# Pitt-JonesLab/slam_decomposition

Hardware: AMD Instinct MI355X
Metric: Haar 2-qubit decompositions/sec (span<=3, loss<1e-8) (higher is better)
Workload: dtype f64

## Files before the change

slam_decomposition_amd/csrc/slam_device.hpp:

```cpp
#pragma once
#include <hip/hip_runtime.h>
#include <stdint.h>

#include "slam_sincos.hpp"
#include "slam_types.hpp"

namespace slamdev {

constexpr int kQuadsPerWave = 16;
constexpr int kWave = 64;
constexpr int kRow = kWave + 1;

typedef float f32x2 __attribute__((ext_vector_type(2)));
typedef float f32x4 __attribute__((ext_vector_type(4)));

template <int K, bool PSQ = false>
struct Cfg {
    static constexpr int L = K + 1;
    static constexpr int N = 6 * L;
    static constexpr int NA = (N + 3) / 4;
    static constexpr int NP = NA * 4;
    static constexpr int NBLK = NA * (NA + 1) / 2;
    static constexpr int FNEED = 20 * NA - 16;
    static constexpr int FSTRIDE = (FNEED - 4 + 31) / 32 * 32 + 4;
    static constexpr int PSP = (N + 3) / 4 * 4 + 1;
    static constexpr int TOFF = PSQ ? 6 : 0;
    static constexpr int PS0 = 12 * K + TOFF;
    static constexpr int XNEED_D = PSQ ? PS0 + 3 * PSP + N : 2 * N;
    static constexpr int XNEED_F = (kQuadsPerWave * FSTRIDE + 2 * kQuadsPerWave - 1) / (2 * kQuadsPerWave);
    static constexpr int XNEED = XNEED_D > XNEED_F ? XNEED_D : XNEED_F;
    static constexpr int XSTRIDE = PSQ ? (XNEED - 4 + 15) / 16 * 16 + 4 : (XNEED - 4 + 7) / 8 * 8 + 4;
    static constexpr int LDS_XCHG = kQuadsPerWave * XSTRIDE;
    static_assert(kQuadsPerWave * FSTRIDE * 4 <= LDS_XCHG * 8, "float overlay must fit the exchange area");
    static constexpr int LDS_FH = 2 * K * 4 * kRow * 2;
    static constexpr int LDS_DOUBLES = LDS_XCHG + LDS_FH;
    static constexpr int LDS_FH_LEAN = (K - 1) * 4 * kRow * 2;
    static constexpr int LDS_DOUBLES_LEAN = LDS_XCHG + LDS_FH_LEAN;
};

template <int K, int GC>
__host__ __device__ constexpr bool lean_layout() { return GC != 0; }
template <int K, int GC>
__host__ __device__ constexpr bool psq_layout() { return lean_layout<K, GC>() && K <= 3; }
template <int K, int GC>
__host__ __device__ constexpr int lds_work_doubles() {
    return lean_layout<K, GC>() ? Cfg<K, psq_layout<K, GC>()>::LDS_DOUBLES_LEAN : Cfg<K, false>::LDS_DOUBLES;
}
constexpr int kColdDoubles = 4;
constexpr int kSincosLdsDoubles = 2 * kSincosTableDoubles;
constexpr int kSeedRing = 8;
constexpr int kSeedRingOff = 70;
template <int K, int GC>
__host__ __device__ constexpr bool seed_ring() { return K == 1 && psq_layout<K, GC>(); }
template <int K, int GC>
__host__ __device__ constexpr int lds_doubles() { return lds_work_doubles<K, GC>() + kSincosLdsDoubles + kColdDoubles; }

__device__ const double kSinCosTable[kSincosTableDoubles] = SLAM_SINCOS_TABLE;

__device__ __forceinline__ void load_sincos_table(double2* tbl, int lane) {
    const double2 t = reinterpret_cast<const double2*>(kSinCosTable)[lane & 31];
    tbl[lane] = (lane & 32) ? make_double2(-t.x, -t.y) : t;
}

typedef const __attribute__((address_space(4))) double* gate_ptr;

__device__ __forceinline__ gate_ptr gate_matrix(const double* gates, int j) {
    unsigned long long a = (unsigned long long)(gates + 32 * j);
    asm volatile("" : "+s"(a));
    return (gate_ptr)a;
}

template <int CTRL>
__device__ __forceinline__ double dpp_f64(double v) {
    int lo = __double2loint(v), hi = __double2hiint(v);
    lo = __builtin_amdgcn_update_dpp(0, lo, CTRL, 0xF, 0xF, true);
    hi = __builtin_amdgcn_update_dpp(0, hi, CTRL, 0xF, 0xF, true);
    return __hiloint2double(hi, lo);
}
template <int CTRL>
__device__ __forceinline__ int dpp_i32(int v) {
    return __builtin_amdgcn_update_dpp(0, v, CTRL, 0xF, 0xF, true);
}
template <int CTRL>
__device__ __forceinline__ double quad_shuffle(double v) { return dpp_f64<CTRL>(v); }
__device__ __forceinline__ double quad_sum(double v) {
    v += quad_shuffle<0xB1>(v);
    v += quad_shuffle<0x4E>(v);
    return v;
}
__device__ __forceinline__ void quad_sum2(double& a, double& b) {
    const double a1 = quad_shuffle<0xB1>(a), b1 = quad_shuffle<0xB1>(b);
    a += a1; b += b1;
    const double a2 = quad_shuffle<0x4E>(a), b2 = quad_shuffle<0x4E>(b);
    a += a2; b += b2;
}
__device__ __forceinline__ double max_abs(double a, double b) {
    double m;
    asm("v_max_f64 %0, |%1|, |%2|" : "=v"(m) : "v"(a), "v"(b));
    return m;
}
__device__ __forceinline__ double quad_max(double v) {
    v = max_abs(v, quad_shuffle<0xB1>(v));
    v = max_abs(v, quad_shuffle<0x4E>(v));
    return v;
}

__device__ __forceinline__ void lds_fence() {
    __builtin_amdgcn_fence(__ATOMIC_RELEASE, "wavefront");
    __builtin_amdgcn_wave_barrier();
    __builtin_amdgcn_fence(__ATOMIC_ACQUIRE, "wavefront");
}

__device__ __forceinline__ void philox4x32_10(uint32_t c0, uint32_t c1, uint32_t c2, uint32_t c3,
                                              uint32_t k0, uint32_t k1, uint32_t (&out)[4]) {
#pragma unroll
    for (int r = 0; r < 10; ++r) {
        const uint64_t p0 = (uint64_t)0xD2511F53u * c0;
        const uint64_t p1 = (uint64_t)0xCD9E8D57u * c2;
        const uint32_t n0 = (uint32_t)(p1 >> 32) ^ c1 ^ k0;
        const uint32_t n1 = (uint32_t)p1;
        const uint32_t n2 = (uint32_t)(p0 >> 32) ^ c3 ^ k1;
        const uint32_t n3 = (uint32_t)p0;
        c0 = n0; c1 = n1; c2 = n2; c3 = n3;
        k0 += 0x9E3779B9u;
        k1 += 0xBB67AE85u;
    }
    out[0] = c0; out[1] = c1; out[2] = c2; out[3] = c3;
}

__device__ __forceinline__ double x0_from_words(uint32_t a, uint32_t b) {
    const uint64_t m = ((uint64_t)(a >> 5) << 26) + (uint64_t)(b >> 6);
    return (double)m * (1.0 / 9007199254740992.0) * 6.283185307179586476925286766559;
}
__device__ __forceinline__ double x0_philox(uint64_t seed, uint32_t target, uint32_t restart, uint32_t k,
                                            uint32_t i) {
    uint32_t w[4];
    philox4x32_10(i >> 1, restart, target, k, (uint32_t)seed, (uint32_t)(seed >> 32), w);
    return (i & 1) ? x0_from_words(w[2], w[3]) : x0_from_words(w[0], w[1]);
}

struct U3t {
    double c, s;
    double cp, sp;
    double cl, sl;
};

__device__ __forceinline__ U3t load_u3(const double* xq, int base_param) {
    const double2* t = reinterpret_cast<const double2*>(xq) + base_param;
    const double2 a = t[0], b = t[1], c = t[2];
    U3t u;
    u.c = a.x; u.s = a.y; u.cp = b.x; u.sp = b.y; u.cl = c.x; u.sl = c.y;
    return u;
}

__device__ __forceinline__ void u3_col(const U3t& t, double& f0r, double& f0i, double& f1r, double& f1i) {
    const double g1r = t.cl * f1r - t.sl * f1i;
    const double g1i = t.cl * f1i + t.sl * f1r;
    const double y0r = t.c * f0r - t.s * g1r;
    const double y0i = t.c * f0i - t.s * g1i;
    const double tr = t.s * f0r + t.c * g1r;
    const double ti = t.s * f0i + t.c * g1i;
    f0r = y0r; f0i = y0i;
    f1r = t.cp * tr - t.sp * ti;
    f1i = t.cp * ti + t.sp * tr;
}

__device__ __forceinline__ void u3_unit(const U3t& t, double f0, double f1, double& y0r, double& y0i, double& y1r, double& y1i) {
    const double g1r = t.cl * f1, g1i = t.sl * f1;
    y0r = t.c * f0 - t.s * g1r;
    y0i = -(t.s * g1i);
    const double tr = t.s * f0 + t.c * g1r;
    const double ti = t.c * g1i;
    y1r = t.cp * tr - t.sp * ti;
    y1i = t.cp * ti + t.sp * tr;
}

__device__ __forceinline__ void u3_unit_t(const U3t& t, double f0, double f1, double& y0r, double& y0i, double& y1r, double& y1i,
                                          double& tr, double& ti) {
// ... 408 lines not shown
        mr[p] = (xr[a] * zr[b] - xi[a] * zi[b]) - (xr[b] * zr[a] - xi[b] * zi[a]);
        mi[p] = (xr[a] * zi[b] + xi[a] * zr[b]) - (xr[b] * zi[a] + xi[b] * zr[a]);
    }
#pragma unroll
    for (int p = 0; p < 6; ++p) { orr[p] = dpp_f64<0x4E>(mr[p]); oi[p] = dpp_f64<0x4E>(mi[p]); }
    const bool hi = q & 2;
    double dr = 0.0, di = 0.0;
#pragma unroll
    for (int p = 0; p < 6; ++p) {
        const double Pr = hi ? orr[p] : mr[p], Pi = hi ? oi[p] : mi[p];
        const double Qr = hi ? mr[5 - p] : orr[5 - p], Qi = hi ? mi[5 - p] : oi[5 - p];
        const double s = (p == 1 || p == 4) ? -1.0 : 1.0;
        dr = fma(s, Pr * Qr - Pi * Qi, dr);
        di = fma(s, Pr * Qi + Pi * Qr, di);
    }
    v.dr = dr; v.di = di;
}

__device__ __forceinline__ void mk_g(const MkInv& v, double (&g)[3], double& idr, double& idi, double& G1r, double& G1i, double& G2r,
                                     double& G2i) {
    const double rd = fast_rcp(v.dr * v.dr + v.di * v.di);
    idr = v.dr * rd; idi = -v.di * rd;
    const double sr = v.tr * v.tr - v.ti * v.ti, si = 2.0 * v.tr * v.ti;
    G1r = 0.0625 * (sr * idr - si * idi); G1i = 0.0625 * (sr * idi + si * idr);
    const double er = sr - v.t2r, ei = si - v.t2i;
    G2r = 0.25 * (er * idr - ei * idi); G2i = 0.25 * (er * idi + ei * idr);
    g[0] = G1r; g[1] = G1i; g[2] = G2r;
}

__device__ __forceinline__ void mk_target_g(const double* tcol, int q, double (&g)[3]) {
    double tr[4], ti[4];
#pragma unroll
    for (int r = 0; r < 4; ++r) {
        const double2 t = *reinterpret_cast<const double2*>(tcol + 8 * r);
        tr[r] = t.x; ti[r] = t.y;
    }
    MkInv v;
    mk_invariants(tr, ti, q, v);
    double a, b, c, d, e, f;
    mk_g(v, g, a, b, c, d, e, f);
}

__device__ __forceinline__ void mk_loss_seed(const double (&wr)[4], const double (&wi)[4], int q, const double (&gT)[3], double& fout,
                                             double (&Ur)[4], double (&Ui)[4]) {
    MkInv v;
    mk_invariants(wr, wi, q, v);
    double g[3], idr, idi, G1r, G1i, G2r, G2i;
    mk_g(v, g, idr, idi, G1r, G1i, G2r, G2i);
    const double D1 = g[0] - gT[0], D2 = g[1] - gT[1], D3 = g[2] - gT[2];
    fout = fma(D1, D1, fma(D2, D2, D3 * D3));
    const double a1r = 2.0 * D1, a1i = -2.0 * D2, a3 = 2.0 * D3;
    const double tdr = v.tr * idr - v.ti * idi, tdi = v.tr * idi + v.ti * idr;
    const double cr = fma(0.125, a1r, 0.5 * a3), ci = 0.125 * a1i;
    const double alr = tdr * cr - tdi * ci, ali = tdr * ci + tdi * cr;
    const double ber = -0.25 * a3 * idr, bei = -0.25 * a3 * idi;
    const double gar = -((a1r * G1r - a1i * G1i) + a3 * G2r), gai = -((a1r * G1i + a1i * G1r) + a3 * G2i);
    double accr[4] = {0.0, 0.0, 0.0, 0.0}, acci[4] = {0.0, 0.0, 0.0, 0.0};
    auto accum = [&](int m, const double (&cr_)[4], const double (&ci_)[4]) {
        const double kr = mk_y(m) * v.br[3 - m], ki = mk_y(m) * v.bi[3 - m];
#pragma unroll
        for (int r = 0; r < 4; ++r) {
            accr[r] = fma(kr, cr_[r], fma(-ki, ci_[r], accr[r]));
            acci[r] = fma(kr, ci_[r], fma(ki, cr_[r], acci[r]));
        }
    };
    { double c0r[4], c0i[4]; mk_bcast_col<0>(wr, wi, c0r, c0i); accum(0, c0r, c0i); }
    { double c1r[4], c1i[4]; mk_bcast_col<1>(wr, wi, c1r, c1i); accum(1, c1r, c1i); }
    { double c2r[4], c2i[4]; mk_bcast_col<2>(wr, wi, c2r, c2i); accum(2, c2r, c2i); }
    { double c3r[4], c3i[4]; mk_bcast_col<3>(wr, wi, c3r, c3i); accum(3, c3r, c3i); }
    double wbr[4], wbi[4];
#pragma unroll
    for (int r = 0; r < 4; ++r) { wbr[r] = dpp_f64<0x1B>(wr[r]); wbi[r] = dpp_f64<0x1B>(wi[r]); }
    const double yq = ((q + 1) & 2) ? 1.0 : -1.0;
#pragma unroll
    for (int c = 0; c < 4; ++c) {
        const double s = yq * mk_y(c);
        const double xr = 2.0 * (alr * wbr[3 - c] - ali * wbi[3 - c]) + 4.0 * (ber * accr[3 - c] - bei * acci[3 - c]);
        const double xi = 2.0 * (alr * wbi[3 - c] + ali * wbr[3 - c]) + 4.0 * (ber * acci[3 - c] + bei * accr[3 - c]);
        Ur[c] = fma(s, xr, gar * wr[c] + gai * wi[c]);
        Ui[c] = fma(s, xi, gai * wr[c] - gar * wi[c]);
    }
}

template <int K, bool HUGE_ARGS, int GC, bool MK = false, bool ROOMY = false>
__device__ __forceinline__ void eval_quad(const double (&xd)[Cfg<K>::NA], const double* tcol,
                                          const double* gates, double* xq, double2* fh, const double2* tbl,
                                          int q, int theta_bits, int cost_kind, double& fout, double (&gd)[Cfg<K>::NA],
                                          double (&Wr)[4], double (&Wi)[4], const double* mkt = nullptr,
                                          const EvalLaneConsts<Cfg<K>::NA>* lc = nullptr) {
    constexpr bool LEAN = lean_layout<K, GC>();
    constexpr bool PSQ = psq_layout<K, GC>();
    using C = Cfg<K, PSQ>;
    static_assert(!ROOMY || (!HUGE_ARGS && !MK), "the hoisted lane constants: the optimizer's BasicCost / SquareCost evaluation only");
    if constexpr (!ROOMY) asm volatile("" : "+v"(theta_bits));
    double* const xt = xq + (PSQ ? (int)((threadIdx.x & 4) + ((threadIdx.x >> 2) & 2)) : 0);
    auto HS = [](int j) constexpr { return LEAN ? j : 2 * j + 1; };
    double tre[4], tim[4];
    if constexpr (!MK) {
#pragma unroll
        for (int r = 0; r < 4; ++r) {
            const double2 t = *reinterpret_cast<const double2*>(tcol + 8 * r);
            tre[r] = t.x;
            tim[r] = t.y;
        }
    }
    {
        double2* t2 = reinterpret_cast<double2*>(xt);
        if constexpr (HUGE_ARGS) {
#pragma unroll
            for (int a = 0; a < C::NA; ++a) {
                const int i = 4 * a + q;
                const int i3 = i - 3 * ((i * 43) >> 7);
                const double arg = (i3 == 0) ? 0.5 * xd[a] : xd[a];
                double s, c;
                sincos_any(arg, tbl, s, c);
                t2[i] = make_double2(c, s);
            }
        } else {
            double rr[C::NA];
            int kk[C::NA];
            double2 tt[C::NA];
            SincosLits L = sincos_lits_device();
            if constexpr (ROOMY) { L.s1 = lc->s1; L.c1 = lc->c1; }
#pragma unroll
            for (int a = 0; a < C::NA; ++a) {
                int hexp;
                if constexpr (ROOMY) hexp = lc->hexp[a];
                else hexp = __builtin_amdgcn_sbfe(theta_bits, a, 1);
                const double arg = __builtin_amdgcn_ldexp(xd[a], hexp);
                sincos_tbl_lookup<true>(arg, tbl, L, rr[a], kk[a], tt[a]);
            }
            __builtin_amdgcn_sched_barrier(0);
#pragma unroll
            for (int a = 0; a < C::NA; ++a) {
                double s, c;
                sincos_tbl_finish<true>(rr[a], kk[a], tt[a], L, s, c);
                t2[4 * a + q] = make_double2(c, s);
            }
        }
    }
    lds_fence();

    double Pr[4], Pi[4];
    double e0[2], e1[2];
    if constexpr (ROOMY) {
        e0[0] = lc->e0[0]; e0[1] = lc->e0[1];
        e1[0] = lc->e1[0]; e1[1] = lc->e1[1];
    } else {
        int qo = q;
        asm volatile("" : "+v"(qo));
        e0[0] = (qo & 1) ? 0.0 : 1.0; e0[1] = (qo & 1) ? 1.0 : 0.0;
        e1[0] = (qo & 2) ? 0.0 : 1.0; e1[1] = (qo & 2) ? 1.0 : 0.0;
    }
    double Fr[4], Fi[4];
#pragma unroll
    for (int r = 0; r < 4; ++r) {
        Fr[r] = (r == q) ? 1.0 : 0.0;
        Fi[r] = 0.0;
    }
    U3t Bn = load_u3(xt, 0), An = load_u3(xt, 3);
#pragma unroll
    for (int j = 0; j <= K; ++j) {
        if (j > 0 && !LEAN) {
#pragma unroll
            for (int r = 0; r < 4; ++r) fh[((2 * (j - 1)) * 4 + r) * kRow] = make_double2(Fr[r], Fi[r]);
        }
        const U3t B = Bn;
        const U3t A = An;
        GateRegs<GC> Gf;
        if (j < K) {
            if constexpr (GC == GC_XRI || GC == GC_XRI1) u3_arrived(B, A);
            Gf = load_gate<GC>(gates, j);
            if constexpr (GC == GC_XRI || GC == GC_XRI1) __builtin_amdgcn_sched_barrier(0);
        }
        double b0r, b0i, b1r, b1i;
        if (j == 0) {
            u3_unit(B, e0[0], e0[1], b0r, b0i, b1r, b1i);
        } else {
            u3_col(B, Fr[0], Fi[0], Fr[1], Fi[1]);
            u3_col(B, Fr[2], Fi[2], Fr[3], Fi[3]);
        }
        if (j < K) {
            Bn = load_u3(xt, 6 * (j + 1));
            An = load_u3(xt, 6 * (j + 1) + 3);
            __builtin_amdgcn_sched_barrier(0);
        }
        if (j == 0) {
            double a0r, a0i, a1r, a1i;
            u3_unit(A, e1[0], e1[1], a0r, a0i, a1r, a1i);
            Fr[0] = a0r * b0r - a0i * b0i; Fi[0] = a0r * b0i + a0i * b0r;
            Fr[1] = a0r * b1r - a0i * b1i; Fi[1] = a0r * b1i + a0i * b1r;
            Fr[2] = a1r * b0r - a1i * b0i; Fi[2] = a1r * b0i + a1i * b0r;
            Fr[3] = a1r * b1r - a1i * b1i; Fi[3] = a1r * b1i + a1i * b1r;
        } else {
            u3_col(A, Fr[0], Fi[0], Fr[2], Fi[2]);
            u3_col(A, Fr[1], Fi[1], Fr[3], Fi[3]);
        }
        if (j < K) {
            if (LEAN && j == K - 1) {
#pragma unroll
                for (int r = 0; r < 4; ++r) { Pr[r] = Fr[r]; Pi[r] = Fi[r]; }
            } else {
#pragma unroll
                for (int r = 0; r < 4; ++r) fh[(HS(j) * 4 + r) * kRow] = make_double2(Fr[r], Fi[r]);
            }
            gate_col<GC>(Gf, Fr, Fi);
        }
    }
#pragma unroll
    for (int r = 0; r < 4; ++r) { Wr[r] = Fr[r]; Wi[r] = Fi[r]; }

    double Ur[4], Ui[4];
    if constexpr (MK) {
        const double gT[3] = {mkt[0], mkt[1], mkt[2]};
        mk_loss_seed(Fr, Fi, q, gT, fout, Ur, Ui);
    } else {
        double pr = 0.0, pi = 0.0;
#pragma unroll
        for (int r = 0; r < 4; ++r) {
            pr = fma(tre[r], Fr[r], fma(tim[r], Fi[r], pr));
            pi = fma(tre[r], Fi[r], fma(-tim[r], Fr[r], pi));
        }
        quad_sum2(pr, pi);
        const double at2 = pr * pr + pi * pi;
        const double rat = (at2 > 1e-300) ? fast_rsqrt(at2) : 0.0;
        const double at = at2 * rat;
        const double basic = 1.0 - 0.25 * at;
        asm volatile("" : "+s"(cost_kind));
        const bool sq = (cost_kind == 1);
        double c0;
        if constexpr (ROOMY) c0 = lc->c0;
        else c0 = sq ? 1.6 : 1.0;
        const double c1 = sq ? -0.8 : 0.0, d1 = sq ? -1.6 : 0.0;
        fout = basic * fma(c1, basic, c0);
        const double inv = (0.25 * rat) * fma(d1, basic, c0);
        const double zr = -pr * inv, zi = pi * inv;
#pragma unroll
        for (int r = 0; r < 4; ++r) {
            Ur[r] = zr * tre[r] + zi * tim[r];
            Ui[r] = zi * tre[r] - zr * tim[r];
        }
    }

// ... 86 lines not shown
            dtheta_dlam_last_real(B, Ur[0], Ui[0], tB01r, tB01i, fr[0], fr[1], th01, la01);
            dtheta_dlam_last_real(B, Ur[2], Ui[2], tB23r, tB23i, fr[2], fr[3], th23, la23);
        }
        part[0] = th01 + th23;
        part[2] = la01 + la23;
        if (j > 0) {
            const double l2 = im_mul(Ur[2], Ui[2], fr[2], fi[2]);
            const double l3 = im_mul(Ur[3], Ui[3], fr[3], fi[3]);
            part[5] = -(l2 + l3);
        } else {
            part[5] = -(Ui[2] * fr[2] + Ui[3] * fr[3]);
        }
        if constexpr (kThetaOut)
            part[3] = 0.5 * thA2;
        else
            part[3] = dtheta_pair(A, Ur[0], Ui[0], Ur[2], Ui[2], fr[0], fi[0], fr[2], fi[2]) +
                      dtheta_pair(A, Ur[1], Ui[1], Ur[3], Ui[3], fr[1], fi[1], fr[3], fi[3]);
        if (kBwdTrigAhead && j > 0) {
            Bn = load_u3(xt, 6 * (j - 1));
            An = load_u3(xt, 6 * (j - 1) + 3);
            __builtin_amdgcn_sched_barrier(0);
        }
        if constexpr (PSQ) {
#pragma unroll
            for (int m = 0; m < 6; ++m) xq[C::PS0 + q * C::PSP + 6 * j + m] = part[m];
        } else {
#pragma unroll
            for (int m = 0; m < 6; ++m) {
                const double ps = part[m] + dpp_f64<0xB1>(part[m]);
                if ((q & 1) == 0) xq[12 * j + 2 * m + (q >> 1)] = ps;
            }
        }
        if (!kBwdTrigAhead && j > 0) {
            An = load_u3(xt, 6 * (j - 1) + 3);
            Bn = load_u3(xt, 6 * (j - 1));
            __builtin_amdgcn_sched_barrier(0);
        }
        if (j > 0) {
            gate_row<GC>(Gb, Ur, Ui);
            if (LEAN) {
#pragma unroll
                for (int r = 0; r < 4; ++r) { Hr[r] = Pr[r]; Hi[r] = Pi[r]; }
            }
        }
    }

    if constexpr (kL0Out) {
        const U3t B = Bn;
        const U3t A = An;
        double b0r, b0i, b1r, b1i, tbr, tbi, a0r, a0i, a1r, a1i, tar, tai;
        u3_unit_t(B, e0[0], e0[1], b0r, b0i, b1r, b1i, tbr, tbi);
        u3_unit_t(A, e1[0], e1[1], a0r, a0i, a1r, a1i, tar, tai);
        const double wB0r = (Ur[0] * a0r - Ui[0] * a0i) + (Ur[2] * a1r - Ui[2] * a1i), wB0i = (Ur[0] * a0i + Ui[0] * a0r) + (Ur[2] * a1i + Ui[2] * a1r);
        const double wB1r = (Ur[1] * a0r - Ui[1] * a0i) + (Ur[3] * a1r - Ui[3] * a1i), wB1i = (Ur[1] * a0i + Ui[1] * a0r) + (Ur[3] * a1i + Ui[3] * a1r);
        const double wA0r = (Ur[0] * b0r - Ui[0] * b0i) + (Ur[1] * b1r - Ui[1] * b1i), wA0i = (Ur[0] * b0i + Ui[0] * b0r) + (Ur[1] * b1i + Ui[1] * b1r);
        const double wA1r = (Ur[2] * b0r - Ui[2] * b0i) + (Ur[3] * b1r - Ui[3] * b1i), wA1i = (Ur[2] * b0i + Ui[2] * b0r) + (Ur[3] * b1i + Ui[3] * b1r);
        double part[6];
        l0_gate_partials(B, e0[0], e0[1], wB0r, wB0i, wB1r, wB1i, b0r, b0i, b1r, b1i, tbr, tbi, part[0], part[1], part[2]);
        l0_gate_partials(A, e1[0], e1[1], wA0r, wA0i, wA1r, wA1i, a0r, a0i, a1r, a1i, tar, tai, part[3], part[4], part[5]);
        if constexpr (PSQ) {
#pragma unroll
            for (int m = 0; m < 6; ++m) xq[C::PS0 + q * C::PSP + m] = part[m];
        } else {
#pragma unroll
            for (int m = 0; m < 6; ++m) {
                const double ps = part[m] + dpp_f64<0xB1>(part[m]);
                if ((q & 1) == 0) xq[2 * m + (q >> 1)] = ps;
            }
        }
    }

    lds_fence();
    {
        if constexpr (PSQ) {
            const double* ps = xq + C::PS0 + q;
            double p0[C::NA], p1[C::NA], p2[C::NA], p3[C::NA];
#pragma unroll
            for (int a = 0; a < C::NA; ++a) {
                p0[a] = ps[4 * a];
                p1[a] = ps[4 * a + C::PSP];
                p2[a] = ps[4 * a + 2 * C::PSP];
                p3[a] = ps[4 * a + 3 * C::PSP];
            }
#pragma unroll
            for (int a = 0; a < C::NA; ++a) gd[a] = (4 * a + q < C::N) ? (p0[a] + p1[a]) + (p2[a] + p3[a]) : 0.0;
        } else {
            const double2* ps2 = reinterpret_cast<const double2*>(xq) + q;
            double2 ps[C::NA];
#pragma unroll
            for (int a = 0; a < C::NA; ++a) ps[a] = ps2[4 * a];
#pragma unroll
            for (int a = 0; a < C::NA; ++a) gd[a] = (4 * a + q < C::N) ? ps[a].x + ps[a].y : 0.0;
        }
    }
    lds_fence();
}

__host__ __device__ constexpr int blk(int a, int b) { return b * (b + 1) / 2 + a; }

template <int NA>
struct HMat {
    f32x2 h[NA * (NA + 1) / 2][2];
};

template <int NA>
__device__ __forceinline__ void h_set_identity_where(HMat<NA>& H, int q, bool where) {
#pragma unroll
    for (int b = 0; b < NA; ++b)
#pragma unroll
        for (int a = 0; a <= b; ++a)
#pragma unroll
            for (int hh = 0; hh < 2; ++hh) {
                f32x2 cur = H.h[blk(a, b)][hh];
                const float id0 = (a == b && 2 * hh == q) ? 1.0f : 0.0f;
                const float id1 = (a == b && 2 * hh + 1 == q) ? 1.0f : 0.0f;
                cur.x = where ? id0 : cur.x;
                cur.y = where ? id1 : cur.y;
                H.h[blk(a, b)][hh] = cur;
            }
}

template <int NA>
__device__ __forceinline__ void h_set_identity(HMat<NA>& H, int q) {
    const f32x2 z = f32x2{0.0f, 0.0f};
    const f32x2 d0 = f32x2{q == 0 ? 1.0f : 0.0f, q == 1 ? 1.0f : 0.0f};
    const f32x2 d1 = f32x2{q == 2 ? 1.0f : 0.0f, q == 3 ? 1.0f : 0.0f};
#pragma unroll
    for (int b = 0; b < NA; ++b)
#pragma unroll
        for (int a = 0; a <= b; ++a) {
            H.h[blk(a, b)][0] = (a == b) ? d0 : z;
            H.h[blk(a, b)][1] = (a == b) ? d1 : z;
        }
}

template <int NA>
__device__ __forceinline__ void h_matvec(const HMat<NA>& H, const double (&vd)[NA], float* xq32, int q,
                                         double (&out)[NA]) {
    float v32[NA];
#pragma unroll
    for (int a = 0; a < NA; ++a) {
        v32[a] = (float)vd[a];
        xq32[4 * a + q] = v32[a];
    }
    lds_fence();
    float* xt = xq32 + 4 * NA - 16;
    f32x2 acc[NA];
#pragma unroll
    for (int a = 0; a < NA; ++a) acc[a] = f32x2{0.0f, 0.0f};
    constexpr bool kBatch = NA <= 8;
    f32x4 vall[NA];
    if constexpr (kBatch) {
#pragma unroll
        for (int b = 0; b < NA; ++b) vall[b] = *reinterpret_cast<const f32x4*>(xq32 + 4 * b);
        __builtin_amdgcn_sched_barrier(0);
    }
#pragma unroll
    for (int b = 0; b < NA; ++b) {
        const f32x4 vb = kBatch ? vall[b] : *reinterpret_cast<const f32x4*>(xq32 + 4 * b);
        const f32x2 vb0 = f32x2{vb.x, vb.y}, vb1 = f32x2{vb.z, vb.w};
        f32x2 t0 = f32x2{0.0f, 0.0f}, t1 = f32x2{0.0f, 0.0f};
#pragma unroll
        for (int a = 0; a <= b; ++a) {
            acc[a] = __builtin_elementwise_fma(H.h[blk(a, b)][0], vb0, acc[a]);
            acc[a] = __builtin_elementwise_fma(H.h[blk(a, b)][1], vb1, acc[a]);
            if (a < b) {
                const f32x2 va = f32x2{v32[a], v32[a]};
                t0 = __builtin_elementwise_fma(H.h[blk(a, b)][0], va, t0);
                t1 = __builtin_elementwise_fma(H.h[blk(a, b)][1], va, t1);
            }
        }
        if (b >= 1) {
            xt[(4 * b + 0) * 4 + q] = t0.x;
            xt[(4 * b + 1) * 4 + q] = t0.y;
            xt[(4 * b + 2) * 4 + q] = t1.x;
            xt[(4 * b + 3) * 4 + q] = t1.y;
        }
    }
    lds_fence();
    f32x4 tall[NA];
    if constexpr (kBatch) {
#pragma unroll
        for (int a = 1; a < NA; ++a) tall[a] = *reinterpret_cast<const f32x4*>(xt + (4 * a + q) * 4);
        __builtin_amdgcn_sched_barrier(0);
    }
#pragma unroll
    for (int a = 0; a < NA; ++a) {
        float o = acc[a].x + acc[a].y;
        if (a >= 1) {
            const f32x4 t = kBatch ? tall[a] : *reinterpret_cast<const f32x4*>(xt + (4 * a + q) * 4);
            o += (t.x + t.y) + (t.z + t.w);
        }
        out[a] = (double)o;
    }
    lds_fence();
}

template <int NA>
__device__ __forceinline__ void h_update_valu(HMat<NA>& H, const float (&s32)[NA], const float (&w32)[NA],
                                              const float (&v32)[NA], float* xq32, int q) {
#pragma unroll
    for (int a = 0; a < NA; ++a) {
        xq32[4 * a + q] = w32[a];
        xq32[4 * NA + 4 * a + q] = s32[a];
    }
    lds_fence();
#pragma unroll
    for (int b = 0; b < NA; ++b) {
        const f32x4 wb = *reinterpret_cast<const f32x4*>(xq32 + 4 * b);
        const f32x4 sb = *reinterpret_cast<const f32x4*>(xq32 + 4 * NA + 4 * b);
        const f32x2 wb0 = f32x2{wb.x, wb.y}, wb1 = f32x2{wb.z, wb.w};
        const f32x2 sb0 = f32x2{sb.x, sb.y}, sb1 = f32x2{sb.z, sb.w};
#pragma unroll
        for (int a = 0; a <= b; ++a) {
            const f32x2 sa = f32x2{s32[a], s32[a]};
            const f32x2 va = f32x2{v32[a], v32[a]};
            f32x2 h0 = H.h[blk(a, b)][0], h1 = H.h[blk(a, b)][1];
            h0 = __builtin_elementwise_fma(va, sb0, h0);
            h1 = __builtin_elementwise_fma(va, sb1, h1);
            h0 = __builtin_elementwise_fma(sa, wb0, h0);
            h1 = __builtin_elementwise_fma(sa, wb1, h1);
            H.h[blk(a, b)][0] = h0;
            H.h[blk(a, b)][1] = h1;
        }
    }
    lds_fence();
}

template <int NA>
__device__ __forceinline__ void h_update_mfma(HMat<NA>& H, const float (&s32)[NA], const float (&w32)[NA],
                                              const float (&v32)[NA]) {
#pragma unroll
    for (int b = 0; b < NA; ++b) {
#pragma unroll
        for (int a = 0; a <= b; ++a) {
            const f32x2 h0 = H.h[blk(a, b)][0], h1 = H.h[blk(a, b)][1];
            f32x4 c = f32x4{h0.x, h0.y, h1.x, h1.y};
            c = __builtin_amdgcn_mfma_f32_4x4x1f32(s32[b], v32[a], c, 0, 0, 0);
            c = __builtin_amdgcn_mfma_f32_4x4x1f32(w32[b], s32[a], c, 0, 0, 0);
            H.h[blk(a, b)][0] = f32x2{c.x, c.y};
            H.h[blk(a, b)][1] = f32x2{c.z, c.w};
        }
    }
}

template <int NA>
__device__ __forceinline__ void h_update(HMat<NA>& H, const float (&s32)[NA], const float (&w32)[NA],
                                         const float (&v32)[NA], float* , int ) {
    h_update_mfma<NA>(H, s32, w32, v32);
}

template <int NA>
__device__ __forceinline__ double qdot(const double (&a)[NA], const double (&b)[NA]) {
    double s = 0.0;
#pragma unroll
    for (int i = 0; i < NA; ++i) s = fma(a[i], b[i], s);
    return quad_sum(s);
}

}
```

slam_decomposition_amd/csrc/slam_kernels.hpp:

```cpp
#pragma once
#include "slam_device.hpp"

namespace slamdev {

constexpr double kArmijoC1 = 1e-4;
constexpr int kMaxBacktrack = 20;
constexpr double kStepMax = 2.0;
constexpr double kCurvEps = 1e-10;
constexpr double kStallDf = 1e-15;
constexpr double kStallGnorm = 1e-5;
constexpr double kWolfeC2 = 0.7;
constexpr double kGrowFactor = 8.0;
constexpr double kGrowMax = 1048576.0;
constexpr int kRestartPeriod = 128;
static_assert((kRestartPeriod & (kRestartPeriod - 1)) == 0, "the periodic restart tests iters & (period - 1)");

__device__ __forceinline__ unsigned long long pack2(int lo, int hi) { return (unsigned long long)(unsigned)lo | ((unsigned long long)(unsigned)hi << 32); }
__device__ __forceinline__ void item_rec_store(ItemRec* r, double loss, int iters, int status, int evals, int acc) {
    r->loss = loss;
    asm volatile("" ::: "memory");
    r->iters = iters;
    asm volatile("" ::: "memory");
    r->status = status;
    asm volatile("" ::: "memory");
// ... 80 lines not shown
        double gT[3];
        mk_target_g(tcol, q, gT);
        eval_quad<K, true, GC, true>(xd, tcol, args.gates, xchg + quad * C::XSTRIDE, fhbase + lane, tbl, q, theta_slot_bits<K>(q), args.cost_kind, f, gd,
                                     Wr, Wi, gT);
    } else {
        eval_quad<K, true, GC>(xd, tcol, args.gates, xchg + quad * C::XSTRIDE, fhbase + lane, tbl, q, theta_slot_bits<K>(q), args.cost_kind, f, gd, Wr, Wi);
    }
    if (live) {
        if (q == 0) args.loss[item] = f;
        if (args.unitary) {
#pragma unroll
            for (int r = 0; r < 4; ++r) {
                args.unitary[item * 32 + (r * 4 + q) * 2] = Wr[r];
                args.unitary[item * 32 + (r * 4 + q) * 2 + 1] = Wi[r];
            }
        }
        if (args.grad) {
#pragma unroll
            for (int a = 0; a < C::NA; ++a) {
                const int i = 4 * a + q;
                if (i < C::N) args.grad[item * C::N + i] = gd[a];
            }
        }
    }
}
template <int K, int GC>
__global__ void __launch_bounds__(kWave) eval_kernel(EvalArgs<K> args) {
    eval_body<K, GC, false>(args);
}
template <int K>
__global__ void __launch_bounds__(kWave) eval_mk_kernel(EvalArgs<K> args) {
    eval_body<K, GC_DENSE, true>(args);
}

template <int K>
__device__ __forceinline__ const __attribute__((address_space(4))) MinimizeArgs<K>* cold_args() {
    unsigned long long a = (unsigned long long)__builtin_amdgcn_kernarg_segment_ptr();
    asm volatile("" : "+s"(a));
    return (const __attribute__((address_space(4))) MinimizeArgs<K>*)a;
}
template <int K, bool MQ>
__device__ __forceinline__ const __attribute__((address_space(4))) MinimizeArgs<K>* cold_args(unsigned long long cur) {
    if constexpr (MQ) {
        unsigned lo = (unsigned)__builtin_amdgcn_readfirstlane((int)(unsigned)cur), hi = (unsigned)__builtin_amdgcn_readfirstlane((int)(unsigned)(cur >> 32));
        unsigned long long u = ((unsigned long long)hi << 32) | lo;
        asm volatile("" : "+s"(u));
        return (const __attribute__((address_space(4))) MinimizeArgs<K>*)u;
    } else {
        return cold_args<K>();
    }
}

struct WlStage {
    int t;
    int* flag;
    double* win_x;
    double win_loss;
    int win_r;
    bool hit;
    unsigned ev_all, ev_acc, ev_pre;
    unsigned rounds;
    unsigned round_cap;
};
__device__ __forceinline__ double readlane_f64(double v, int l) {
    const int lo = __builtin_amdgcn_readlane(__double2loint(v), l), hi = __builtin_amdgcn_readlane(__double2hiint(v), l);
    return __hiloint2double(hi, lo);
}

template <int K, int GC, bool MQ, bool WL, bool MK = false>
__device__ __forceinline__ void minimize_body(const MinimizeArgs<K>& args, const MinimizeArgs<K>* subs, int n_sub, WlStage& wl) {
    static_assert(!WL || MQ, "the wave-local stage reads its argument block from device memory");
    static_assert(!MK || (!MQ && GC == GC_DENSE), "MakhlinFunctionalCost: per-span launches of the dense gate class only");
    using C = Cfg<K, psq_layout<K, GC>()>;
    constexpr int NA = C::NA;
    extern __shared__ __attribute__((aligned(16))) double lds[];
    double* xchg = lds;
    double2* fhbase = reinterpret_cast<double2*>(lds + C::LDS_XCHG);
    const int lane = threadIdx.x;
    int q = lane & 3;
    const int quad = lane >> 2;
    const int theta_bits = theta_slot_bits<K>(q);
    constexpr bool kRoomy = roomy_regs<K, GC, MQ, WL>() && !MK;
    constexpr bool kRoomyItem = kRoomy && !MQ;
    EvalLaneConsts<NA> lane_consts;
    if constexpr (kRoomy) eval_lane_consts<K>(q, args.cost_kind, lane_consts);
    double* xq = xchg + quad * C::XSTRIDE;
    float* xq32 = reinterpret_cast<float*>(xchg) + quad * C::FSTRIDE;
    double2* fh = fhbase + lane;
    double2* tbl = reinterpret_cast<double2*>(lds + lds_work_doubles<K, GC>());
    load_sincos_table(tbl, lane);
    double2* cold = tbl + kSincosLdsDoubles / 2;
    if (lane == 0) {
        cold[0] = make_double2(args.gtol, args.stop_loss);
        cold[1] = make_double2(args.gtol_far, args.far_loss);
    }
    lds_fence();
    constexpr bool kRing = seed_ring<K, GC>();
    if constexpr (kRing) static_assert(kSeedRingOff + C::N <= C::XSTRIDE && kSeedRingOff >= C::XNEED && (kSeedRingOff & 1) == 0, "the ring slots sit in the spare part of a quad's exchange area");
    double* const ring = xchg + 8 * C::XSTRIDE + kSeedRingOff;
    unsigned ring_base = 0, ring_end = 0;
    unsigned sub_idx = MQ ? (unsigned)blockIdx.x % (unsigned)n_sub : 0u;
    unsigned long long cur = MQ ? (unsigned long long)(subs + sub_idx) : 0ull;
    int sub_tries = 0;
    unsigned n_act = WL ? 1u : (unsigned)(MQ ? cold_args<K, MQ>(cur)->ctl->n_active : args.ctl->n_active);
    unsigned n_items = n_act * (unsigned)args.restarts;
    unsigned n_waves = (n_items + kQuadsPerWave - 1) / kQuadsPerWave;
    if constexpr (WL) {
        n_waves = 1;
    } else if constexpr (!MQ) {
        if (args.items_per_quad > 1) {
            n_waves = (n_items + kQuadsPerWave * args.items_per_quad - 1) / (kQuadsPerWave * args.items_per_quad);
            if (n_waves < 1 && n_items) n_waves = 1;
        }
        if (n_waves > gridDim.x) n_waves = gridDim.x;
        if (blockIdx.x >= n_waves) return;
    } else {
        n_waves = gridDim.x / (unsigned)n_sub + 1u;
    }
    unsigned kChunkV;
    {
        const unsigned per_wave = n_items / n_waves;
        kChunkV = per_wave >= 256u ? 64u : (per_wave >= 64u ? 32u : 16u);
    }

    bool live = false, fresh = false, scaled = false;
    unsigned item = 0;
    int slot = 0, tgt = 0;
    int nev = 0, iters = 0, nback = 0, nstall = 0, status = ST_MAXITER;
    double f = 0.0, alpha = 0.0, gp = 0.0, gnorm = 0.0, grow = 1.0;
    double pp = 0.0, hs1 = 0.0;
    const double* tcol = cold_args<K, MQ>(cur)->targets + q * 2;
    const int32_t* sflag_ptr = nullptr;
    int beat_level = 0;
    if constexpr (kRoomyItem) sflag_ptr = args.solved;
    double x[NA], g[NA], p[NA];
#pragma unroll
    for (int a = 0; a < NA; ++a) { x[a] = 0.0; g[a] = 0.0; p[a] = 0.0; }
    HMat<NA> H;
    h_set_identity_where<NA>(H, q, true);
    double mkt[3] = {0.0, 0.0, 0.0};
    bool exhausted = false;
    const unsigned kChunk = kChunkV;
    unsigned cur_next = 0, cur_end = WL ? n_items : 0u;
    unsigned pre_base = 0;
    unsigned rounds = 0;
    if constexpr (!WL) {
        if (lane == 0) pre_base = atomicAdd(&cold_args<K, MQ>(cur)->ctl->work_counter, kChunk);
    }

    while (true) {
        if constexpr (MQ && !WL) {
            if (exhausted && !__any(live)) {
                if (lane == 0 && rounds) atomicAdd(&cold_args<K, MQ>(cur)->ctl->rounds, (unsigned long long)rounds);
                rounds = 0;
                if (++sub_tries >= n_sub) break;
                sub_idx = (sub_idx + 1u == (unsigned)n_sub) ? 0u : sub_idx + 1u;
                cur = (unsigned long long)(subs + sub_idx);
                n_act = (unsigned)cold_args<K, MQ>(cur)->ctl->n_active;
                n_items = n_act * (unsigned)args.restarts;
                exhausted = false;
                cur_next = 0;
                cur_end = 0;
                ring_base = 0;
                ring_end = 0;
                if (lane == 0) pre_base = atomicAdd(&cold_args<K, MQ>(cur)->ctl->work_counter, kChunk);
            }
// ... 125 lines not shown
                            }
                        }
#pragma unroll
                        for (int a = 0; a < NA; ++a) {
                            p[a] = 0.0;
                            g[a] = 0.0;
                        }
                        alpha = 0.0; gp = 0.0; f = 0.0; grow = 1.0; pp = 0.0; hs1 = 0.0;
                        nev = 0; iters = 0; nback = 0; nstall = 0; status = ST_MAXITER;
                        scaled = false; fresh = true; live = true; taken = true;
                        h_set_identity<NA>(H, q);
                    }
                    if constexpr (kRing) {
                        if (shared && get) {
#pragma unroll
                            for (int a = 0; a < NA; ++a) x[a] = (4 * a + q < C::N) ? ring[rslot * C::XSTRIDE + 4 * a + q] : 0.0;
                        }
                    } else if constexpr (kSharedSeeds) {
                        if (shared) {
                            constexpr int kPairs = C::N / 2;
                            static_assert(5 * C::N <= C::XSTRIDE && 4 * C::N * 8 >= 64 * 4, "staging area [4N, 5N) inside the quad's exchange area and clear of wp");
                            if (get && q == 0) {
                                wp[32 + qrank] = tgt + (int)cold_args<K, MQ>(cur)->target_base;
                                wp[48 + qrank] = quad;
                            }
                            lds_fence();
                            const uint64_t seed = cold_args<K, MQ>(cur)->seed;
                            const int jobs = n_take * kPairs;
                            for (int j0 = 0; j0 < jobs; j0 += kWave) {
                                const int jb = j0 + lane;
                                if (jb < jobs) {
                                    const int r = jb / kPairs, m = jb - r * kPairs;
                                    uint32_t w[4];
                                    philox4x32_10((uint32_t)m, (uint32_t)wp[16 + r], (uint32_t)wp[32 + r], (uint32_t)K, (uint32_t)seed,
                                                  (uint32_t)(seed >> 32), w);
                                    *reinterpret_cast<double2*>(xchg + wp[48 + r] * C::XSTRIDE + 4 * C::N + 2 * m) =
                                        make_double2(x0_from_words(w[0], w[1]), x0_from_words(w[2], w[3]));
                                }
                            }
                            lds_fence();
                            if (get) {
#pragma unroll
                                for (int a = 0; a < NA; ++a) x[a] = (4 * a + q < C::N) ? xq[4 * C::N + 4 * a + q] : 0.0;
                            }
                            lds_fence();
                        }
                    }
                    if ((args.flags & kFlagNoExterior) && get) {
#pragma unroll
                        for (int a = 0; a < NA; ++a) {
                            const int i = 4 * a + q;
                            x[a] = (i < 6 || i >= 6 * K) ? 0.0 : x[a];
                        }
                    }
                }
            }
            if constexpr (MK) {
                if (__any(taken)) {
                    double g3[3];
                    mk_target_g(tcol, q, g3);
#pragma unroll
                    for (int i = 0; i < 3; ++i) mkt[i] = taken ? g3[i] : mkt[i];
                }
            }
        }
        if (!__any(live)) {
            if constexpr (MQ && !WL) continue;
            else break;
        }
        if constexpr (WL) {
            if (rounds >= wl.round_cap) break;
        }
        ++rounds;

        int sflag = 0;
        if (args.flags & 1u) {
            if constexpr (WL) sflag = *reinterpret_cast<volatile int*>(wl.flag);
            else if constexpr (kRoomyItem) sflag = __hip_atomic_load(sflag_ptr, __ATOMIC_RELAXED, __HIP_MEMORY_SCOPE_AGENT);
            else sflag = __hip_atomic_load(&(MQ ? cold_args<K, MQ>(cur)->solved : args.solved)[slot], __ATOMIC_RELAXED, __HIP_MEMORY_SCOPE_AGENT);
        }

        double gt[NA];
        double ft, Wr[4], Wi[4];
        {
            double xt[NA];
#pragma unroll
            for (int a = 0; a < NA; ++a) xt[a] = fma(alpha, p[a], x[a]);
            if constexpr (MK) {
                eval_quad<K, false, GC, true>(xt, tcol, args.gates, xq, fh, tbl, q, theta_bits, 0, ft, gt, Wr, Wi, mkt);
            } else {
                eval_quad<K, false, GC, false, kRoomy>(xt, tcol, MQ ? cold_args<K, MQ>(cur)->gates : args.gates, xq, fh, tbl, q, theta_bits,
                                                       WL ? __builtin_amdgcn_readfirstlane(args.cost_kind) : args.cost_kind, ft, gt, Wr, Wi, nullptr,
                                                       kRoomy ? &lane_consts : nullptr);
            }
        }
        const bool active = live;
        const bool finite = isfinite(ft);
#pragma unroll
        for (int a = 0; a < NA; ++a) gt[a] = finite ? gt[a] : 0.0;
        if (args.flags & kFlagNoExterior) {
#pragma unroll
            for (int a = 0; a < NA; ++a) {
                const int i = 4 * a + q;
                gt[a] = (i < 6 || i >= 6 * K) ? 0.0 : gt[a];
            }
        }
        const bool armijo = finite && (ft <= f + kArmijoC1 * alpha * gp);
        const bool acc = active && (fresh ? finite : armijo);
        const bool step = acc && !fresh;
        nev += active ? (acc ? 0x100001 : 1) : 0;

        const double am = step ? alpha : 0.0;
        double qv[NA];
        __builtin_amdgcn_sched_barrier(0);
        h_matvec<NA>(H, gt, xq32, q, qv);
        __builtin_amdgcn_sched_barrier(0);
        double pgt = 0.0, yy = 0.0;
#pragma unroll
        for (int a = 0; a < NA; ++a) {
            const double ya = gt[a] - g[a];
            pgt = fma(p[a], gt[a], pgt);
            yy = fma(ya, ya, yy);
        }
        quad_sum2(pgt, yy);
        const double sg = am * pgt;
        const double sy = am * (pgt - gp);
        const double ss = (am * am) * pp;
        const bool too_short = sy < (1.0 - kWolfeC2) * alpha * (-gp);
        const bool curv = step && !too_short && sy > 0.0 && (sy * sy > (kCurvEps * kCurvEps) * (ss * yy));
        const bool first = curv && !scaled;
        scaled = scaled || curv;
        const double fac = first ? (sy * fast_rcp(yy)) : 1.0;
        hs1 = first ? fac - 1.0 : hs1;
        double yu = 0.0;
#pragma unroll
        for (int a = 0; a < NA; ++a) {
            qv[a] = fma(hs1, gt[a], qv[a]);
            const double ua = fma(fac, p[a], qv[a]);
            yu = fma(gt[a] - g[a], ua, yu);
        }
        yu = quad_sum(yu);
        const double rho = curv ? fast_rcp(sy) : 0.0;
        const double cf = rho * (1.0 + rho * yu);
        double wg = 0.0;
        {
            float s32[NA], w32[NA], v32[NA];
#pragma unroll
            for (int a = 0; a < NA; ++a) {
                const double sa = am * p[a];
                const double ua = fma(fac, p[a], qv[a]);
                const double wa = cf * sa - rho * ua;
                const double va = -rho * ua;
                s32[a] = (float)sa;
                w32[a] = (float)wa;
                v32[a] = (float)va;
                wg = fma(wa, gt[a], wg);
            }
            __builtin_amdgcn_sched_barrier(0);
            h_update<NA>(H, s32, w32, v32, xq32, q);
            __builtin_amdgcn_sched_barrier(0);
        }
        wg = quad_sum(wg);
        const double2 th0 = cold[0], th1 = cold[1];
        __builtin_amdgcn_sched_barrier(0);

#pragma unroll
        for (int a = 0; a < NA; ++a) x[a] += am * p[a];
        bool done = false;
        if (acc) {
            nstall = (step && (f - ft) <= kStallDf) ? nstall + 1 : 0;
            f = ft;
            if (step) ++iters;
            nback = 0;
            grow = (step && too_short) ? fmin(grow * kGrowFactor, kGrowMax) : 1.0;
#pragma unroll
            for (int a = 0; a < NA; ++a) {
                const double sa = am * p[a];
                const double ua = fma(fac, p[a], qv[a]);
                const double va = -rho * ua;
                g[a] = gt[a];
                p[a] = -(qv[a] + sa * wg + va * sg);
            }
            if (args.flags & kFlagTrace) {
                const auto* ca = cold_args<K, MQ>(cur);
                const int t_cap = ca->trace_cap;
                double* const t_loss = ca->trace_loss;
                double* const t_x = ca->trace_x;
                if (step && iters <= t_cap) {
                const int64_t row = (int64_t)item * t_cap + (iters - 1);
                if (q == 0) t_loss[row] = f;
#pragma unroll
                for (int a = 0; a < NA; ++a) {
                    const int i = 4 * a + q;
                    if (i < C::N) t_x[row * C::N + i] = x[a];
                }
                }
            }
        } else if (active) {
            if (fresh) {
                f = ft;
                status = ST_NONFINITE;
                done = true;
            } else {
                const double denom = 2.0 * (ft - f - gp * alpha);
                const double anew = (finite && denom > 0.0 && isfinite(denom)) ? (-gp * alpha * alpha * fast_rcp(denom)) : 0.5 * alpha;
                alpha = fmin(fmax(anew, 0.1 * alpha), 0.5 * alpha);
                grow = 1.0;
                ++nback;
            }
        }
        {
            double m = max_abs(g[0], g[NA > 1 ? 1 : 0]);
#pragma unroll
            for (int a = 2; a < NA; ++a) m = max_abs(m, g[a]);
            gnorm = quad_max(m);
        }
        gp = qdot<NA>(g, p);
        pp = qdot<NA>(p, p);
        if (acc) {
            alpha = (pp > 1e-300) ? fmin(grow, kStepMax * fast_rsqrt(pp)) : grow;
            if (f < th0.y || gnorm < th0.x || (gnorm < th1.x && f > th1.y)) {
                status = ST_CONVERGED; done = true;
            } else if (nstall >= 2) { status = ST_STALLED; done = true; }
            else if (iters >= args.maxiter) { status = ST_MAXITER; done = true; }
        } else if (active && !fresh) {
            if (nback > kMaxBacktrack) { status = (gnorm < kStallGnorm) ? ST_STALLED : ST_LINESEARCH; done = true; }
        }
        fresh = false;
        const bool periodic = step && !done && ((iters & (kRestartPeriod - 1)) == 0);
        const bool reset = active && !done && (!(gp < 0.0) || periodic);
        if (__any(reset)) {
            h_set_identity_where<NA>(H, q, reset);
            hs1 = reset ? 0.0 : hs1;
            scaled = periodic ? false : scaled;
#pragma unroll
            for (int a = 0; a < NA; ++a) p[a] = reset ? -g[a] : p[a];
            const double gg2 = qdot<NA>(g, g);
            gp = reset ? -gg2 : gp;
            pp = reset ? gg2 : pp;
            alpha = periodic ? ((gg2 > 1e-300) ? fmin(grow, kStepMax * fast_rsqrt(gg2)) : grow) : alpha;
        }
        if (args.flags & 1u) {
            asm volatile("" : "+v"(sflag));
            if constexpr (kRoomyItem) {
                if (active && !done && sflag > beat_level) { status = ST_PREEMPTED; done = true; }
                if (active && done && status != ST_PREEMPTED && f < args.exit_loss && q == 0) {
                    const int mine = args.restarts - (int)(item - (unsigned)slot * (unsigned)args.restarts);
                    __hip_atomic_fetch_max(&args.solved[slot], mine, __ATOMIC_RELAXED, __HIP_MEMORY_SCOPE_AGENT);
                }
            } else {
                const int mine = args.restarts - (int)(item - (unsigned)slot * (unsigned)args.restarts);
                const bool beaten = (args.flags & 2u) ? (sflag > mine) : (sflag != 0);
                if (active && !done && beaten) { status = ST_PREEMPTED; done = true; }
// ... 567 lines not shown
```

Measured before the change: 4.779 million.

## Hide LDS latency by interleaving line-search bookkeeping and trig exchange in eval

For small K with the PSQ layout, the line-search acceptance logic (Armijo test, step counters, x update) is moved into a callback that runs while the gradient partial-sum LDS loads are in flight. The sincos finish is split so the layer-0 U3 values are written, fenced and loaded before the remaining angles finish. For K=1, the dot products and the first quad-reduction stage are also placed under the outstanding LDS loads in h_matvec. The goal is to fill LDS latency bubbles with independent ALU work, at the cost of an extra wave fence and possibly more register pressure.

```diff
diff --git a/slam_decomposition_amd/csrc/slam_device.hpp b/slam_decomposition_amd/csrc/slam_device.hpp
--- a/slam_decomposition_amd/csrc/slam_device.hpp
+++ b/slam_decomposition_amd/csrc/slam_device.hpp
@@ -1,6 +1,8 @@
 #pragma once
 #include <hip/hip_runtime.h>
 #include <stdint.h>
+
+#include <type_traits>
 
 #include "slam_sincos.hpp"
 #include "slam_types.hpp"
@@ -94,6 +96,20 @@
     const double a2 = quad_shuffle<0x4E>(a), b2 = quad_shuffle<0x4E>(b);
     a += a2; b += b2;
 }
+__device__ __forceinline__ void quad_sum2_stage1(double& a, double& b) {
+    const double a1 = quad_shuffle<0xB1>(a), b1 = quad_shuffle<0xB1>(b);
+    a += a1; b += b1;
+}
+__device__ __forceinline__ void quad_sum2_stage2(double& a, double& b) {
+    const double a2 = quad_shuffle<0x4E>(a), b2 = quad_shuffle<0x4E>(b);
+    a += a2; b += b2;
+}
+struct NoFill {
+    __device__ __forceinline__ void operator()() const {}
+    __device__ __forceinline__ void operator()(double) const {}
+};
+template <class F>
+inline constexpr bool has_fill = !std::is_same<F, NoFill>::value;
 __device__ __forceinline__ double max_abs(double a, double b) {
     double m;
     asm("v_max_f64 %0, |%1|, |%2|" : "=v"(m) : "v"(a), "v"(b));
@@ -668,12 +684,13 @@
     }
 }
 
-template <int K, bool HUGE_ARGS, int GC, bool MK = false, bool ROOMY = false>
+template <int K, bool HUGE_ARGS, int GC, bool MK = false, bool ROOMY = false, bool SPLIT = false, class UnderGrad = NoFill>
 __device__ __forceinline__ void eval_quad(const double (&xd)[Cfg<K>::NA], const double* tcol,
                                           const double* gates, double* xq, double2* fh, const double2* tbl,
                                           int q, int theta_bits, int cost_kind, double& fout, double (&gd)[Cfg<K>::NA],
                                           double (&Wr)[4], double (&Wi)[4], const double* mkt = nullptr,
-                                          const EvalLaneConsts<Cfg<K>::NA>* lc = nullptr) {
+                                          const EvalLaneConsts<Cfg<K>::NA>* lc = nullptr, UnderGrad under_grad = {}) {
+    static_assert(!SPLIT || (!HUGE_ARGS && Cfg<K>::NA > 2), "the split trig exchange: the table-lookup form, layer 0 in slots 0 and 1");
     constexpr bool LEAN = lean_layout<K, GC>();
     constexpr bool PSQ = psq_layout<K, GC>();
     using C = Cfg<K, PSQ>;
@@ -690,6 +707,7 @@
             tim[r] = t.y;
         }
     }
+    U3t Bn, An;
     {
         double2* t2 = reinterpret_cast<double2*>(xt);
         if constexpr (HUGE_ARGS) {
@@ -717,11 +735,30 @@
                 sincos_tbl_lookup<true>(arg, tbl, L, rr[a], kk[a], tt[a]);
             }
             __builtin_amdgcn_sched_barrier(0);
+            if constexpr (SPLIT) {
+#pragma unroll
+                for (int a = 0; a < 2; ++a) {
+                    double s, c;
+                    sincos_tbl_finish<true>(rr[a], kk[a], tt[a], L, s, c);
+                    t2[4 * a + q] = make_double2(c, s);
+                }
+                lds_fence();
+                Bn = load_u3(xt, 0);
+                An = load_u3(xt, 3);
+                __builtin_amdgcn_sched_barrier(0);
+#pragma unroll
+                for (int a = 2; a < C::NA; ++a) {
+                    double s, c;
+                    sincos_tbl_finish<true>(rr[a], kk[a], tt[a], L, s, c);
+                    t2[4 * a + q] = make_double2(c, s);
+                }
+            } else {
 #pragma unroll
             for (int a = 0; a < C::NA; ++a) {
                 double s, c;
                 sincos_tbl_finish<true>(rr[a], kk[a], tt[a], L, s, c);
                 t2[4 * a + q] = make_double2(c, s);
+            }
             }
         }
     }
@@ -744,7 +781,10 @@
         Fr[r] = (r == q) ? 1.0 : 0.0;
         Fi[r] = 0.0;
     }
-    U3t Bn = load_u3(xt, 0), An = load_u3(xt, 3);
+    if constexpr (!SPLIT) {
+        Bn = load_u3(xt, 0);
+        An = load_u3(xt, 3);
+    }
 #pragma unroll
     for (int j = 0; j <= K; ++j) {
         if (j > 0 && !LEAN) {
@@ -997,6 +1037,12 @@
                 p2[a] = ps[4 * a + 2 * C::PSP];
                 p3[a] = ps[4 * a + 3 * C::PSP];
             }
+            if constexpr (has_fill<UnderGrad>) {
+                asm volatile("" : "+v"(fout));
+                __builtin_amdgcn_sched_barrier(0);
+                under_grad(fout);
+                __builtin_amdgcn_sched_barrier(0);
+            }
 #pragma unroll
             for (int a = 0; a < C::NA; ++a) gd[a] = (4 * a + q < C::N) ? (p0[a] + p1[a]) + (p2[a] + p3[a]) : 0.0;
         } else {
@@ -1049,9 +1095,10 @@
         }
 }
 
-template <int NA>
+template <int NA, class UnderV = NoFill, class UnderT = NoFill>
 __device__ __forceinline__ void h_matvec(const HMat<NA>& H, const double (&vd)[NA], float* xq32, int q,
-                                         double (&out)[NA]) {
+                                         double (&out)[NA], UnderV under_v = {}, UnderT under_t = {}) {
+    static_assert((!has_fill<UnderV> && !has_fill<UnderT>) || NA <= 8, "the fills sit behind the batched requests");
     float v32[NA];
 #pragma unroll
     for (int a = 0; a < NA; ++a) {
@@ -1069,6 +1116,10 @@
 #pragma unroll
         for (int b = 0; b < NA; ++b) vall[b] = *reinterpret_cast<const f32x4*>(xq32 + 4 * b);
         __builtin_amdgcn_sched_barrier(0);
+        if constexpr (has_fill<UnderV>) {
+            under_v();
+            __builtin_amdgcn_sched_barrier(0);
+        }
     }
 #pragma unroll
     for (int b = 0; b < NA; ++b) {
@@ -1098,6 +1149,10 @@
 #pragma unroll
         for (int a = 1; a < NA; ++a) tall[a] = *reinterpret_cast<const f32x4*>(xt + (4 * a + q) * 4);
         __builtin_amdgcn_sched_barrier(0);
+        if constexpr (has_fill<UnderT>) {
+            under_t();
+            __builtin_amdgcn_sched_barrier(0);
+        }
     }
 #pragma unroll
     for (int a = 0; a < NA; ++a) {
diff --git a/slam_decomposition_amd/csrc/slam_kernels.hpp b/slam_decomposition_amd/csrc/slam_kernels.hpp
--- a/slam_decomposition_amd/csrc/slam_kernels.hpp
+++ b/slam_decomposition_amd/csrc/slam_kernels.hpp
@@ -186,6 +186,8 @@
     const int theta_bits = theta_slot_bits<K>(q);
     constexpr bool kRoomy = roomy_regs<K, GC, MQ, WL>() && !MK;
     constexpr bool kRoomyItem = kRoomy && !MQ;
+    constexpr bool kOrder = K <= 2 && psq_layout<K, GC>() && !WL && !MK;
+    constexpr bool kLossUnder = kOrder, kTrigSplit = kOrder, kSumsUnder = kOrder && K == 1;
     EvalLaneConsts<NA> lane_consts;
     if constexpr (kRoomy) eval_lane_consts<K>(q, args.cost_kind, lane_consts);
     double* xq = xchg + quad * C::XSTRIDE;
@@ -477,20 +479,38 @@
 
         double gt[NA];
         double ft, Wr[4], Wi[4];
+        const bool active = live;
+        bool e_finite = false, e_acc = false, e_step = false;
+        double e_am = 0.0;
+        int e_nstall = 0;
         {
             double xt[NA];
 #pragma unroll
             for (int a = 0; a < NA; ++a) xt[a] = fma(alpha, p[a], x[a]);
             if constexpr (MK) {
                 eval_quad<K, false, GC, true>(xt, tcol, args.gates, xq, fh, tbl, q, theta_bits, 0, ft, gt, Wr, Wi, mkt);
+            } else if constexpr (kLossUnder) {
+                auto loss_only = [&](double ftv) {
+                    e_finite = isfinite(ftv);
+                    const bool armijo = e_finite && (ftv <= f + kArmijoC1 * alpha * gp);
+                    e_acc = active && (fresh ? e_finite : armijo);
+                    e_step = e_acc && !fresh;
+                    nev += active ? (e_acc ? 0x100001 : 1) : 0;
+                    e_am = e_step ? alpha : 0.0;
+#pragma unroll
+                    for (int a = 0; a < NA; ++a) x[a] += e_am * p[a];
+                    e_nstall = (e_step && (f - ftv) <= kStallDf) ? nstall + 1 : 0;
+                };
+                eval_quad<K, false, GC, false, kRoomy, kTrigSplit>(xt, tcol, MQ ? cold_args<K, MQ>(cur)->gates : args.gates, xq, fh, tbl, q, theta_bits,
+                                                                   WL ? __builtin_amdgcn_readfirstlane(args.cost_kind) : args.cost_kind, ft, gt, Wr, Wi,
+                                                                   nullptr, kRoomy ? &lane_consts : nullptr, loss_only);
             } else {
-                eval_quad<K, false, GC, false, kRoomy>(xt, tcol, MQ ? cold_args<K, MQ>(cur)->gates : args.gates, xq, fh, tbl, q, theta_bits,
-                                                       WL ? __builtin_amdgcn_readfirstlane(args.cost_kind) : args.cost_kind, ft, gt, Wr, Wi, nullptr,
-                                                       kRoomy ? &lane_consts : nullptr);
-            }
-        }
-        const bool active = live;
-        const bool finite = isfinite(ft);
+                eval_quad<K, false, GC, false, kRoomy, kTrigSplit>(xt, tcol, MQ ? cold_args<K, MQ>(cur)->gates : args.gates, xq, fh, tbl, q, theta_bits,
+                                                                   WL ? __builtin_amdgcn_readfirstlane(args.cost_kind) : args.cost_kind, ft, gt, Wr, Wi,
+                                                                   nullptr, kRoomy ? &lane_consts : nullptr);
+            }
+        }
+        const bool finite = kLossUnder ? e_finite : isfinite(ft);
 #pragma unroll
         for (int a = 0; a < NA; ++a) gt[a] = finite ? gt[a] : 0.0;
         if (args.flags & kFlagNoExterior) {
@@ -501,23 +521,37 @@
             }
         }
         const bool armijo = finite && (ft <= f + kArmijoC1 * alpha * gp);
-        const bool acc = active && (fresh ? finite : armijo);
-        const bool step = acc && !fresh;
-        nev += active ? (acc ? 0x100001 : 1) : 0;
-
-        const double am = step ? alpha : 0.0;
+        const bool acc = kLossUnder ? e_acc : active && (fresh ? finite : armijo);
+        const bool step = kLossUnder ? e_step : acc && !fresh;
+        if constexpr (!kLossUnder) nev += active ? (acc ? 0x100001 : 1) : 0;
+
+        const double am = kLossUnder ? e_am : (step ? alpha : 0.0);
         double qv[NA];
+        double pgt = 0.0, yy = 0.0;
         __builtin_amdgcn_sched_barrier(0);
-        h_matvec<NA>(H, gt, xq32, q, qv);
-        __builtin_amdgcn_sched_barrier(0);
-        double pgt = 0.0, yy = 0.0;
-#pragma unroll
-        for (int a = 0; a < NA; ++a) {
-            const double ya = gt[a] - g[a];
-            pgt = fma(p[a], gt[a], pgt);
-            yy = fma(ya, ya, yy);
-        }
-        quad_sum2(pgt, yy);
+        if constexpr (kSumsUnder) {
+            auto products = [&]() {
+#pragma unroll
+                for (int a = 0; a < NA; ++a) {
+                    const double ya = gt[a] - g[a];
+                    pgt = fma(p[a], gt[a], pgt);
+                    yy = fma(ya, ya, yy);
+                }
+            };
+            h_matvec<NA>(H, gt, xq32, q, qv, products, [&]() { quad_sum2_stage1(pgt, yy); });
+            __builtin_amdgcn_sched_barrier(0);
+            quad_sum2_stage2(pgt, yy);
+        } else {
+            h_matvec<NA>(H, gt, xq32, q, qv);
+            __builtin_amdgcn_sched_barrier(0);
+#pragma unroll
+            for (int a = 0; a < NA; ++a) {
+                const double ya = gt[a] - g[a];
+                pgt = fma(p[a], gt[a], pgt);
+                yy = fma(ya, ya, yy);
+            }
+            quad_sum2(pgt, yy);
+        }
         const double sg = am * pgt;
         const double sy = am * (pgt - gp);
         const double ss = (am * am) * pp;
@@ -559,11 +593,14 @@
         const double2 th0 = cold[0], th1 = cold[1];
         __builtin_amdgcn_sched_barrier(0);
 
-#pragma unroll
-        for (int a = 0; a < NA; ++a) x[a] += am * p[a];
+        if constexpr (!kLossUnder) {
+#pragma unroll
+            for (int a = 0; a < NA; ++a) x[a] += am * p[a];
+        }
         bool done = false;
         if (acc) {
-            nstall = (step && (f - ft) <= kStallDf) ? nstall + 1 : 0;
+            if constexpr (kLossUnder) nstall = e_nstall;
+            else nstall = (step && (f - ft) <= kStallDf) ? nstall + 1 : 0;
             f = ft;
             if (step) ++iters;
             nback = 0;
```

After: 4.855 million (median of 6 runs). +1.6%, better.
